# davidmilligan/MLVFS

Measured on AMD Instinct MI355X. Metric: Mpix/s, 3584x1320 14-bit unpack+badpix+cs5x5+stripes (fused, stream resident in HBM), higher is better.
Workload: dtype u16/int32

## Files before the change

### include/mlvfs_amd.h

```cpp
#ifndef MLVFS_AMD_H
#define MLVFS_AMD_H

#include <stddef.h>
#include <stdint.h>
#include <sys/types.h>

#include "mlvfs_abi.h"

#ifdef __cplusplus
extern "C" {
#endif


size_t dng_get_image_data(struct frame_headers *frame_headers, uint16_t *packed_bits,
                          uint8_t *output_buffer, off_t offset, size_t max_size);
size_t dng_get_header_data(struct frame_headers *frame_headers, uint8_t *output_buffer, off_t offset, size_t max_size,
                           double fps_override, char *mlv_basename);
size_t mlvfs_amd_dng_header_lossless(struct frame_headers *frame_headers, uint8_t *output_buffer, off_t offset, size_t max_size,
                                     double fps_override, const char *mlv_basename, uint32_t stream_bytes);
size_t dng_get_header_size(void);
size_t dng_get_image_size(struct frame_headers *frame_headers);
size_t dng_get_size(struct frame_headers *frame_headers);

void chroma_smooth(struct frame_headers *frame_headers, uint16_t *image_data, int method);
// ... 150 lines not shown
int mlvfs_amd_hdr_preview_dev(const mlvfs_amd_geom_t *geom, void *d_frame, size_t max_size, void *stream);

int mlvfs_amd_deflicker_dev(const mlvfs_amd_geom_t *geom, const void *d_frame, size_t size_bytes, int target,
                            int32_t exposure_bias[2], void *stream);

int mlvfs_amd_cr2hdr20_dev(const mlvfs_amd_geom_t *geom, void *d_frame, int interp_method, int fullres, int use_alias_map,
                           int chroma_smooth, void *stream);
int mlvfs_amd_cr2hdr20_batch_dev(const mlvfs_amd_geom_t *geom, void *d_frames, size_t stride, int nframes, int interp_method,
                                 int fullres, int use_alias_map, int chroma_smooth, int *results, void *stream);
void mlvfs_amd_dualiso_reset(void);
void mlvfs_amd_dualiso_trim(void);
void mlvfs_amd_dualiso_last_scalars(double out[8]);

int mlvfs_amd_amaze_demosaic_dev(const float *d_raw, int width, int height, float *d_red, float *d_green, float *d_blue, void *stream);
void mlvfs_amd_amaze_rows_extent(int width, int height, int *nfx, int *nfy);
int mlvfs_amd_amaze_rows_extra_mode(int mode, int width, int height, int *count);
int mlvfs_amd_amaze_debug(const float *d_raw, int width, int height, float *d_red, float *d_green, float *d_blue, int mode,
                          float *d_planes, size_t planes_floats, int *nfx, int *nfy);

int mlvfs_amd_timer_begin(int max_launches);
int mlvfs_amd_timer_end(float *ms, int cap);

int mlvfs_amd_frame_begin(void);
int mlvfs_amd_frame_end(void);
int mlvfs_amd_frame_sync(void *image_data);
void mlvfs_amd_dropin_stats(long long out[2]);
void mlvfs_amd_dropin_transfers(long long out[4]);
void mlvfs_amd_dropin_profile(double out[8]);
void mlvfs_amd_test_fail_next(int what);
int mlvfs_amd_test_rand_layout(void);
int mlvfs_amd_test_device_order(const char *const *bus_ids, int n, int workers, int *device_of);

int mlvfs_amd_test_stream_plan(int width, int height, int seg_rows, int *cols, int *segs, int *fold, int *tasks_per_frame);
int mlvfs_amd_test_frame_plan(const int *in, long long *out);
int mlvfs_amd_test_last_frame_plan(long long out[15]);
int mlvfs_amd_test_stream_listed(void *stream, long long *tiles);
int mlvfs_amd_test_dualiso_parts(int width, int height, int nframes, int *parts, int max_parts, int *tail);

int mlvfs_amd_fix_pattern_noise_dev(const mlvfs_amd_geom_t *geom, void *d_frames, size_t stride, int nframes, void *stream);
size_t mlvfs_amd_test_pn_scratch_cap(size_t bytes);
int mlvfs_amd_deflicker_batch_dev(const mlvfs_amd_geom_t *geom, const void *d_frames, size_t stride, int nframes, size_t size_bytes,
                                  int target, int32_t *exposure_bias, void *stream);
int mlvfs_amd_hdr_preview_batch_dev(const mlvfs_amd_geom_t *geom, void *d_frames, size_t stride, int nframes, size_t max_size,
                                    int *results, void *stream);

typedef struct {
    int32_t chroma_smooth;
    int32_t fix_bad_pixels;
    int32_t fix_stripes;
    int32_t dual_iso;
    int32_t hdr_interpolation_method;
    int32_t hdr_no_fullres;
    int32_t hdr_no_alias_map;
    int32_t deflicker;
    int32_t fix_pattern_noise;
    int32_t rand_mode;
    double fps;
} mlvfs_amd_mount_opts_t;
void *mlvfs_amd_mount_open(const void *reader, const mlvfs_amd_mount_opts_t *opts, const char *mlv_basename);
int mlvfs_amd_mount_dng(void *mount, int first, int count, void *h_out, size_t out_stride, int batch_frames, int io_threads, int *results);
int mlvfs_amd_mount_dng_lossless(void *mount, int first, int count, void *h_out, size_t out_stride, size_t *sizes, int *flags,
                                 int batch_frames, int io_threads, int *results);
void mlvfs_amd_mount_close(void *mount);

typedef struct mlvfs_amd_dark mlvfs_amd_dark_t;
typedef struct mlvfs_amd_look mlvfs_amd_look_t;
typedef struct mlvfs_amd_look16 mlvfs_amd_look16_t;
mlvfs_amd_dark_t *mlvfs_amd_dark_create(const mlvfs_amd_geom_t *geom, const uint16_t *h_plane);
mlvfs_amd_dark_t *mlvfs_amd_dark_from_clip(const void *reader, int first, int count, int batch_frames, int io_threads);
// ... 177 lines not shown
```

### mlvfs_amd/csrc/clip.h

```cpp
#pragma once

#include "common.h"

#include <algorithm>
#include <functional>
#include <memory>
#include <mutex>
#include <vector>

namespace mlv {

constexpr int FRAME_TCW = 64, FRAME_TCH = 15, FRAME_TCH5 = 15, FRAME_HC = 2;
constexpr int FRAME_GEOS = 2;
inline int frame_tile_rows(int geo) { return geo == 1 ? FRAME_TCH5 : FRAME_TCH; }
inline int frame_geo_of(int method) { return method == 5 ? 1 : 0; }
inline int frame_tiles_x(int w) { return (w + 2 * FRAME_TCW - 1) / (2 * FRAME_TCW); }
inline int frame_tiles_y(int h, int geo) { return (h + 2 * frame_tile_rows(geo) - 1) / (2 * frame_tile_rows(geo)); }

struct CellRec {
    int cell;
    int e[4];
};

struct PatchView {
// ... 54 lines not shown
    Geom g{};
    int row0 = 0, row1 = 0, gpr = 0, n_groups = 0, nblk = 0;
    size_t o_counts = 0, o_bsum = 0, o_boff = 0, o_total = 0, o_hist = 0, o_num = 0, o_nre = 0, o_re = 0, o_copies = 0, bytes = 0;
    uint8_t *base = nullptr;
    int init(Clip *owner, const Geom &g, int row0, int row1);
    int count(const void *d_frame, long long *accepted, hipStream_t stream);
    int hist_dev(const void *d_frame, const void *d_rand, long long n_rand, int *d_hist, int *d_num, hipStream_t stream);
    int recheck_into(int32_t *hist_host_or_null, int *d_hist, hipStream_t stream);
    int hist_to_host(const void *d_frame, const void *d_rand, long long n_rand, int32_t *hist, int32_t num[8],
                     hipStream_t stream);
};

struct ThreadCtx;
bool focus_map_applies(struct frame_headers *fh, ThreadCtx *c, int dual_iso);
int focus_pixels_device(struct frame_headers *fh, ThreadCtx *c, void *d_frame, int dual_iso, bool *changed, int *n_patched = nullptr);
int bad_pixels_device(struct frame_headers *fh, ThreadCtx *c, void *d_frame, int aggressive, int dual_iso, bool *changed, int *n_patched = nullptr);

void glibc_rand_stream(uint16_t *out, size_t n, uint64_t skip, unsigned seed);
int stripes_solve(const int32_t *hist, const int32_t num[8], int frame_size, int32_t coeffs[8]);

struct KernelTimer {
    std::vector<hipEvent_t> ev;
    int used = 0;
    bool on = false;
};
KernelTimer &kernel_timer();

int launch_unpack(const void *d_packed, size_t packed_stride, void *d_out, size_t out_stride, uint32_t first_px,
                  uint32_t npix, int bpp, int nframes, hipStream_t stream);
int launch_frame(const Device *dev, const Geom &g, bool packed, const void *src, size_t src_stride, void *dst,
                 size_t dst_stride, int nframes, int method, const PatchView *pv, bool stripes,
                 const int32_t *coef, hipStream_t stream, bool spread = false);
int stream_listed_tiles(hipStream_t stream, long long *tiles);
int dark_share(int packed_bpp, const void *d_frame, int w, int h, int black, hipStream_t stream, int *share_1024);
bool frame_kernel_takes(const Geom &g, const void *src, size_t src_stride, const void *dst, size_t dst_stride, int nframes);
int launch_pixfix(int packed, const void *frames, size_t stride, int w, int black, const void *entries,
                  const int *level_off, int n_levels, int n_level0, int n_entries, void *patches, void *scatter,
                  size_t scatter_stride, int nframes, const DeviceLuts &luts, hipStream_t stream);
int launch_pixfix_for_frame_kernel(int packed, const void *frames, size_t stride, int w, int h, int black, const void *entries,
                                   const int *level_off, int n_levels, int n_level0, int n_entries, void *patches,
                                   const CellRec *recs, int n_rec, void *cells, int nframes, const DeviceLuts &luts, hipStream_t stream);
int launch_pixfix_cells(int packed, const void *frames, size_t stride, int w, int h, const CellRec *recs, int n_rec,
                        const void *patches, int n_entries, void *cells, int nframes, hipStream_t stream);
int launch_deflicker_hist(const void *d_frame, uint32_t samples, uint32_t white, unsigned *d_hist, hipStream_t s);
int launch_deflicker_batch(const void *d_frames, size_t fstride, int nframes, uint32_t samples, uint32_t white, uint32_t middle, unsigned *d_hist,
                           uint16_t *d_med, hipStream_t s);
struct HdrPreviewParams {
    double a, b;
    int dark_row_start, shadow, active, pad;
};
int launch_hdr_row_hist_batch(const void *d_frames, size_t fstride, int nframes, int w, int h, int white, unsigned *d_hist, hipStream_t stream);
int launch_hdr_preview_batch(const void *d_frames, void *d_out, size_t fstride, int nframes, int w, int h, int black, int white,
                             const HdrPreviewParams *d_params, size_t shift_count, hipStream_t stream);
size_t pattern_noise_batch_frame_bytes(int w, int h);
size_t pattern_noise_scratch_cap();
int launch_pattern_noise_batch(void *d_frames, size_t fstride, int nframes, int w, int h, int white, void *d_scratch, size_t scratch_bytes,
                               hipStream_t stream);
int hdr_preview_batch_device(ThreadCtx *c, const Geom &g, void *d_frames, void *d_out, size_t fstride, int nframes, size_t max_size,
                             unsigned *d_hist, HdrPreviewParams *d_params, struct frame_headers *fhs, int *results, hipStream_t stream);
int deflicker_batch_device(const void *d_frames, size_t fstride, int nframes, int bpp, size_t size_bytes, void *d_scratch, size_t scratch_bytes,
                           uint16_t *med, hipStream_t stream);
size_t deflicker_batch_scratch_bytes(int bpp, int nframes);
void deflicker_bias(int target, int black_level, uint16_t median, int32_t exposure_bias[2]);
enum { PAYLOAD_PLAIN = 0, PAYLOAD_LZMA = 1, PAYLOAD_LJ92 = 2 };
inline int payload_kind(uint16_t video_class) { return (video_class & 0x80) ? PAYLOAD_LZMA : (video_class & 0x100) ? PAYLOAD_LJ92 : PAYLOAD_PLAIN; }
struct Calib {
// ... 72 lines not shown
```

### mlvfs_amd/csrc/frame_plan.cpp

```cpp
#include "frame_plan.h"

#include "clip.h"

namespace mlv {

namespace {
constexpr int WGS_PER_CU = 4;
constexpr int RUN_MAX = 22;
constexpr int P5_SEG = 60;
constexpr int S_SEG = 60;

int cus(const FramePassInputs &in) { return in.num_cu > 0 ? in.num_cu : 256; }

int env_switch(const char *name) { const char *e = getenv(name); return e ? atoi(e) : 1; }

bool streamable(const FramePassInputs &in)
{
    return in.packed && in.bpp == 14 && (in.vec == 1 || in.vec == 2) && in.black >= 0 && in.black <= 16384 && in.stripes != StripeForm::generic &&
           in.w >= 16 && in.w % 8 == 0 && in.h >= 2 && in.h % 2 == 0;
}

bool s_takes(const FramePassInputs &in, const FrameSwitches &sw)
{
    if ((in.method != 2 && in.method != 3) || sw.s == 0 || in.pixel_map || !streamable(in)) return false;
    const StreamGeom g = stream_geom(in.w, in.h, S_SEG);
    const long long waves = (long long)cus(in) * WGS_PER_CU * 4;
    return sw.s == 2 || (long long)in.nframes * g.cols * g.segs * 2 >= waves * 7;
}

int p5_seg_rows(const FramePassInputs &in, const FrameSwitches &sw, int grid)
{
    if (in.method != 5 || sw.p5 == 0 || !streamable(in)) return 0;
    const long long cols = stream_geom(in.w, in.h, P5_SEG).cols, rows = in.h / 2;
    const long long waves = (long long)(grid / 4 > 0 ? grid / 4 : 256) * 16;
    for (int seg : { P5_SEG, P5_SEG / 2 })
// ... 38 lines not shown
}

int plan_frame_pass(const FramePassInputs &in, const FrameSwitches &sw, const StreamVerdict &v, FramePlan *out)
{
    if (const int rc = check_frame_pass(in)) return rc;
    FramePlan p;
    const int tiles_x = frame_tiles_x(in.w);
    p.tiles = (long long)tiles_x * frame_tiles_y(in.h, frame_geo_of(in.method)) * in.nframes;

    p.grid = (cus(in) * WGS_PER_CU + 7) / 8 * 8;
    if (p.grid > p.tiles) p.grid = (int)((p.tiles + 7) / 8 * 8);
    const int per_cu = std::min(std::max(p.grid / 4, 1), FRAME_MAX_GROUPS);
    p.groups = per_cu >= 64 ? per_cu / 8 / 8 * 8 : per_cu;
    const int band = (int)(p.tiles / p.groups);
    p.run = std::min(std::max(band / 16, 1), RUN_MAX);
    p.singles = p.run > 1 ? 8 * std::max(p.grid / p.groups, 1) : 0;

    p.watch = frame_pass_watch(in, sw);
    const bool held = p.watch.adaptive && v.held;
    if (p.watch.word == 1 && !held) {
        p.first = FirstKernel::s;
        p.seg_rows = S_SEG;
    } else if (p.watch.word == 0 && !held) {
        p.list_after = true;
        p.seg_rows = v.some_listed && sw.p5 != 2 ? 0 : p5_seg_rows(in, sw, p.grid);
        p.first = p.seg_rows ? FirstKernel::p5 : FirstKernel::p;
        p.first_grid = p.grid;
    }
    if (p.seg_rows) {
        const StreamGeom g = stream_geom(in.w, in.h, p.seg_rows);
        p.cols = g.cols; p.segs = g.segs; p.fold = g.fold;
        p.tasks = (long long)in.nframes * g.tasks_per_frame;
    }
    if (p.first == FirstKernel::s) {
        p.first_grid = cus(in) * WGS_PER_CU;
        if ((long long)p.first_grid * 4 > p.tasks) p.first_grid = (int)((p.tasks + 3) / 4);
        p.steps = (long long)in.nframes * ((p.cols - 1) * p.fold + 1) * (in.h / 2) / p.fold;
    }
    if (p.list_after) {
        long long most = p.tiles;
        if (p.first == FirstKernel::p5) {
            const int full_cols = p.fold > 1 ? p.cols - 1 : p.cols, folded = p.fold > 1 ? (p.segs + p.fold - 1) / p.fold : 0;
            const long long per_frame = (long long)full_cols * p.segs * std::min(tiles_x, tile_cols_spanned(4 * 64)) +
                                        (long long)folded * p.fold * std::min(tiles_x, tile_cols_spanned(4 * 64 / p.fold));
            most = std::max(most, in.nframes * per_frame);
        }
        p.wl_entries = std::max(most, 4096ll);
    }
    *out = p;
    return MLVFS_AMD_OK;
}

namespace {
struct LastPlan { FramePlan plan; bool set = false; };
LastPlan &last_plan() { static thread_local LastPlan t; return t; }

void plan_fields(const FramePlan &p, long long *out)
{
    const long long o[15] = { (long long)p.first, p.list_after, p.grid, p.groups, p.run, p.singles, p.first_grid,
                              p.seg_rows, p.cols, p.segs, p.fold, p.tasks, p.steps, p.wl_entries, p.watch.word };
    for (int i = 0; i < 15; i++) out[i] = o[i];
}
}

void record_frame_plan(const FramePlan &p) { LastPlan &l = last_plan(); l.plan = p; l.set = true; }

}

extern "C" int mlvfs_amd_test_stream_plan(int width, int height, int seg_rows, int *cols, int *segs, int *fold, int *tasks_per_frame)
{
    if (width < 16 || width % 8 || height < 2 || height % 2 || seg_rows < 1 || !cols || !segs || !fold || !tasks_per_frame) return MLVFS_AMD_ERR_ARG;
    const mlv::StreamGeom g = mlv::stream_geom(width, height, seg_rows);
    *cols = g.cols; *segs = g.segs; *fold = g.fold; *tasks_per_frame = g.tasks_per_frame;
    return MLVFS_AMD_OK;
}

extern "C" int mlvfs_amd_test_frame_plan(const int *in, long long *out)
{
    if (!in || !out) return MLVFS_AMD_ERR_ARG;
    const mlv::FramePassInputs fi{ in[0], in[1], in[2], in[3], in[4], in[5] != 0, in[6], in[7] != 0,
                                   in[8] == 2 ? mlv::StripeForm::generic : in[8] == 1 ? mlv::StripeForm::packed : mlv::StripeForm::none,
                                   in[9], in[10] };
    const mlv::StreamVerdict v{ in[11] != 0, in[12] != 0 };
    mlv::FramePlan p;
    if (const int rc = mlv::plan_frame_pass(fi, mlv::frame_switches(), v, &p)) return rc;
    mlv::plan_fields(p, out);
    return MLVFS_AMD_OK;
}

extern "C" int mlvfs_amd_test_stream_listed(void *stream, long long *tiles)
{
    return tiles ? mlv::stream_listed_tiles((hipStream_t)stream, tiles) : MLVFS_AMD_ERR_ARG;
}

extern "C" int mlvfs_amd_test_last_frame_plan(long long *out)
{
    const mlv::LastPlan &l = mlv::last_plan();
    if (!out || !l.set) return MLVFS_AMD_ERR_ARG;
    mlv::plan_fields(l.plan, out);
    return MLVFS_AMD_OK;
}
```

### mlvfs_amd/csrc/frame_plan.h

```cpp
#pragma once

namespace mlv {

constexpr int FRAME_STREAM_COLW = 62;
constexpr int FRAME_MAX_GROUPS = 1024;

enum class FirstKernel { none, p, p5, s };
enum class StripeForm { none, packed, generic };

struct FramePassInputs {
    int w, h, bpp, black;
    int method;
    bool packed;
    int vec;
    bool pixel_map;
    StripeForm stripes;
    int nframes, num_cu;
};

struct FrameSwitches { int p = 1, p5 = 1, s = 1; };
FrameSwitches frame_switches();

struct FrameWatch {
    int word = -1;
    bool adaptive = false;
    bool status = false;
};
FrameWatch frame_pass_watch(const FramePassInputs &in, const FrameSwitches &sw);

struct StreamVerdict {
    bool held = false;
    bool some_listed = false;
};

struct StreamGeom { int cols, segs, fold, tasks_per_frame; };
StreamGeom stream_geom(int w, int h, int seg_rows);

struct FramePlan {
    FirstKernel first = FirstKernel::none;
    bool list_after = false;
    FrameWatch watch;
    long long tiles = 0;
    int grid = 0, groups = 0, run = 0, singles = 0;
    int first_grid = 0;
    int seg_rows = 0, cols = 0, segs = 0, fold = 0;
    long long tasks = 0;
    long long steps = 0;
    long long wl_entries = 0;
};

int check_frame_pass(const FramePassInputs &in);
int plan_frame_pass(const FramePassInputs &in, const FrameSwitches &sw, const StreamVerdict &v, FramePlan *out);

void record_frame_plan(const FramePlan &p);

}
```

### mlvfs_amd/csrc/k_frame.hip

```cpp
#include "frame_plan.h"
#include "k_frame_dev.h"

namespace mlv {

template <int METHOD, bool PACKED, int VEC, bool SPREAD>
__global__ __launch_bounds__(256, 4) void k_frame(const FrameArgs a)
{
    constexpr bool CHAIN = METHOD == 5;
    using Smem = SmemT<SPREAD, CHAIN>;
    __shared__ Smem sm;

    const int list_mode = a.list_mode;
    const int wl_n = list_mode ? cold_args()->wl_ctl[0] : 0;
    auto list_done = [&]() {
        KArgs ka = cold_args();
        int *ctl = ka->wl_ctl, *stat = ka->wl_stat;
        if (atomicAdd(&ctl[2], 1) == min((int)gridDim.x, wl_n) - 1) {
            ctl[0] = 0; ctl[1] = 0; ctl[2] = 0;
            if (stat) { __atomic_store_n(stat, ctl[3], __ATOMIC_RELAXED); __threadfence_system(); }
        }
    };
    if (list_mode && (int)blockIdx.x >= wl_n) {
        if (wl_n == 0 && blockIdx.x == 0 && threadIdx.x == 0) {
            KArgs ka = cold_args();
// ... 375 lines not shown
    if (wt.adaptive && st.h_stat) {
        Backoff &b = st.back[wt.word];
        long long reported = 0, of = 0;
        if (b.look(__atomic_load_n(&st.h_stat[wt.word], __ATOMIC_RELAXED), &reported, &of)) {
            b.judge(reported * 100 > of * (wt.word == 0 ? KF_P_BUSY_PERCENT : KF_S_BUSY_PERCENT));
            if (wt.word == 0) st.some_listed = reported * 100 > of * KF_P5_CALM_PERCENT;
        }
        v.held = b.wide_left > 0;
    }
    v.some_listed = st.some_listed;
    if (const int rc = plan_frame_pass(in, sw, v, pl)) return rc;
    if (wt.adaptive && v.held) st.back[wt.word].wide_left--;
    if (pl->list_after && pl->wl_entries > st.wl_cap) {
        if (st.wl) (void)hipFree(st.wl);
        st.wl = nullptr; st.wl_cap = 0;
        if (hipMalloc(&st.wl, (size_t)pl->wl_entries * sizeof(int2)) != hipSuccess) { set_error("work list: allocation of %lld entries failed", pl->wl_entries); return MLVFS_AMD_ERR_HIP; }
        st.wl_cap = pl->wl_entries;
    }
    if (pl->first == FirstKernel::s) st.back[1].pending += pl->steps;
    if (pl->list_after) st.back[0].pending += pl->tiles;
    *out = st;
    return MLVFS_AMD_OK;
}
int stream_listed_tiles(hipStream_t stream, long long *tiles)
{
    int dev = 0;
    if (hipGetDevice(&dev) != hipSuccess) return MLVFS_AMD_ERR_HIP;
    std::lock_guard<std::mutex> lk(g_ticket_mu);
    const auto it = g_tickets.find({ dev, stream });
    if (it == g_tickets.end() || !it->second.h_stat) return MLVFS_AMD_ERR_ARG;
    *tiles = (long long)(unsigned)__atomic_load_n(&it->second.h_stat[0], __ATOMIC_RELAXED);
    return MLVFS_AMD_OK;
}
void release_stream_state(int device, hipStream_t stream)
{
    std::lock_guard<std::mutex> lk(g_ticket_mu);
    auto it = g_tickets.find({ device, stream });
    if (it == g_tickets.end()) return;
    if (it->second.tickets) (void)hipFree(it->second.tickets);
    if (it->second.wl) (void)hipFree(it->second.wl);
    if (it->second.h_stat) (void)hipHostFree(it->second.h_stat);
    g_tickets.erase(it);
}
__global__ __launch_bounds__(256) void k_build_e2d(const uint16_t *__restrict__ u16, int black, uint2 *__restrict__ e2d, int *__restrict__ bad)
{
    const int b = blockIdx.x * blockDim.x + threadIdx.x;
    if (b >= E2D_RECORDS_EXT) return;
    auto entry = [&](int i) { return (uint16_t)((((int)u16[i & 32767]) >> (13 - (i >> 15))) + black); };
    if (b >= E2D_RECORDS) { e2d[b] = make_uint2(entry(E2R_ENTRIES - 1), 0u); return; }
    unsigned bits = 0;
    uint16_t prev = entry(32 * b);
    const uint16_t base = prev;
    for (int j = 0; j < 31; j++) {
        const uint16_t next = entry(32 * b + j + 1);
        const unsigned d = (uint16_t)(next - prev);
        if (d > 1) atomicAdd(bad, 1);
        bits |= (d & 1u) << j;
        prev = next;
    }
    e2d[b] = make_uint2(base, bits);
}
namespace {
constexpr size_t E2R_CACHE = 8;
struct E2rEntry { uint2 *table; unsigned long long used; };
std::mutex g_tables_mu;
std::map<std::pair<int, int>, E2rEntry> g_e2r;
// ... 179 lines not shown
```

### mlvfs_amd/csrc/k_frame_p.hip

```cpp
#include "frame_plan.h"
#include "k_stream_dev.h"

namespace mlv {

constexpr int P_WAIT_MIN = 1, P_WAIT_MAX = 15;
template <bool SPREAD_>
struct __align__(16) SmemP {
    static constexpr bool SPREAD = SPREAD_;
    uint16_t raw[2 * RH][2 * TCW];
    uint32_t pk[PH][PW];
    int ge[RH][TCW];
    uint16_t t16[MLV_T16_N + (SPREAD_ ? 64 : 0)];
    uint32_t has_patch[PMAP_WORDS];
    uint32_t xchg[3][XCHG_WORDS];
    int unc[2];
    int low[2];
    int dim[2];
    int next_tile, next_end;
    int walk[5];
    int2 carry_at[256];
    uint4 carry_spare;
};

struct PGroup {
// ... 522 lines not shown
            fb_wait = min(2 * fb_wait + 1, P_WAIT_MAX);
            cont = false;
        } else {
            fb_wait = P_WAIT_MIN;
            cont = cont_next;
        }
        low_prev = low_cur;
        t = t_next;
        t_end = t_end_next;
        cur = nxt;
        par ^= 1;
    }
    if (tid == 0) {
        KArgs ka = cold_args();
        const int groups = ka->groups;
        int *tickets = ka->tickets;
        if (atomicAdd(&tickets[2 * groups], 1) == (int)gridDim.x - 1)
            for (int i = 0; i <= 2 * groups; i++) tickets[i] = 0;
    }
}

template <bool SPREAD, int VEC>
__global__ __launch_bounds__(1024, 1) void k_frame_p5(const FrameArgs a, int cols, int segs, int seg_rows, int fold, int S_OUT)
{
    static_assert(!SPREAD, "one table layout");
    asm volatile("" : "+s"(cols));
    constexpr int BPP = 14;
    constexpr int WAVES = 16;
    constexpr int SLOTS = 3;
    constexpr int PARK_LANES = 62;
    struct __align__(16) Smem {
        int ev[MLV_EV32_N];
        uint4 park[WAVES][SLOTS][2][PARK_LANES];
    };
    static_assert(sizeof(Smem) <= 160 * 1024, "the CU's LDS");
    __shared__ Smem sm;
    {
        const uint4 *s4 = (const uint4 *)cold_args()->ev32;
        uint4 *d4 = (uint4 *)sm.ev;
        for (int i = (int)threadIdx.x; i < MLV_EV32_N * 4 / 16; i += 64 * WAVES) d4[i] = s4[i];
    }
    __syncthreads();
    const int lane = (int)threadIdx.x & 63;
    const int w = a.w, h = a.h, black = a.black;
    const uint32_t koff = 4u - 4u * (uint32_t)black;
    const int rows = h >> 1;
    const StreamGrid sg = stream_grid(cols, segs, fold);
    const int ntasks = cold_args()->nframes * sg.per_frame;
    const uint32_t pitch = (uint32_t)(w >> 3) * 14u;
    int *tickets = cold_args()->tickets;
    uint4 (*const mypark)[2][PARK_LANES] = sm.park[threadIdx.x >> 6];
    const int plane = min(max(lane - 1, 0), PARK_LANES - 1);
    const bool parks = lane >= 1 && lane <= PARK_LANES;
    for (;;) {
        const int task = stream_draw(tickets, lane);
        if (task >= ntasks) break;
        const StreamTask t = stream_task<VEC>(task, sg, segs, seg_rows, fold, S_OUT, lane, w, rows);
        const int f = t.f, c = t.c, j0 = t.j0, j1 = t.j1, nparts = t.nparts, P = t.P, roff = t.roff;
        KArgs kt = cold_args();
        const uint8_t *const frame = kt->src + (size_t)f * kt->src_stride;
        const mlv_i32x4 rs_in = frame_rsrc(frame, kt->src_bytes);
        mlv_i32x4 rs_out = { 0, 0, 0, 0 };
        int tx0 = 0;
        bool xm = false;
        uint32_t dA0[4], dA1[4], dB0[4], dB1[4];
        auto issue = [&](int r, uint32_t (&d0)[4], uint32_t (&d1)[4]) { stream_issue(rs_in, r, roff, rows, pitch, t.gbyte, d0, d1); };
        issue(j0 - 2, dA0, dA1);
        issue(j0 - 1, dB0, dB1);
        int ref_r, ref_b;
        {
            const int x0 = min(max(8 * (c * S_OUT + S_OUT / 2), 0), (w - 16) & ~1), y0 = min(j0 + j1, (h - 4) & ~1) & ~1;
            const uint32_t px = fetch_clamped<BPP>(frame, w, h, x0 + (lane & 15), y0 + (lane >> 4));
            const int ev = sm.ev[1 + min(max((int)px - black, 1), 16383)];
            constexpr int CX[5] = { 0, 3, 6, 1, 5 }, CY[5] = { 0, 0, 0, 1, 1 };
            int sdr[5], sdb[5];
#pragma unroll
            for (int k = 0; k < 5; k++) {
                const int l0 = 2 * CX[k] + 32 * CY[k];
                const int rr = __builtin_amdgcn_readlane(ev, l0), g1 = __builtin_amdgcn_readlane(ev, l0 + 1);
                const int g2 = __builtin_amdgcn_readlane(ev, l0 + 16), bb = __builtin_amdgcn_readlane(ev, l0 + 17);
                const int gg = (g1 + g2) >> 1;
                sdr[k] = rr - gg; sdb[k] = bb - gg;
            }
            auto med5 = [](const int (&v)[5]) { return med3i(v[4], max(min(v[0], v[1]), min(v[2], v[3])), min(max(v[0], v[1]), max(v[2], v[3]))); };
            ref_r = med5(sdr);
            ref_b = med5(sdb);
        }
        int n_pm = 0, pm_cell = -1;
// ... 233 lines not shown
```

### mlvfs_amd/csrc/k_stream_dev.h

```cpp
#pragma once
#include "k_frame_dev.h"

namespace mlv {

struct StreamGrid { int ncols_full, nfolded, per_frame; };
__device__ __forceinline__ StreamGrid stream_grid(int cols, int segs, int fold)
{
    StreamGrid sg;
    sg.ncols_full = fold > 1 ? cols - 1 : cols;
    sg.nfolded = fold > 1 ? (segs + fold - 1) / fold : 0;
    sg.per_frame = sg.ncols_full * segs + sg.nfolded;
    return sg;
}

__device__ __forceinline__ int stream_draw(int *tickets, int lane)
{
    int task = 0;
    if (lane == 0) task = atomicAdd(&tickets[0], 1);
    return __builtin_amdgcn_readfirstlane(task);
}

struct StreamTask {
    int f, c;
    int j0, j1;
    int nparts, P;
    int pl, part, roff;
    int g;
    bool writes;
    uint32_t gbyte;
    uint32_t sel, sel1;
};
template <int VEC>
__device__ __forceinline__ StreamTask stream_task(int task, const StreamGrid &sg, int segs, int seg_rows, int fold, int S_OUT, int lane, int w, int rows)
{
    StreamTask t;
    const int gmax = (w >> 3) - 1;
    t.f = task / sg.per_frame;
    const int rem = task - t.f * sg.per_frame;
    const bool folded = rem >= sg.ncols_full * segs;
    t.c = folded ? sg.ncols_full : rem / segs;
    const int seg = folded ? (rem - sg.ncols_full * segs) * fold : rem - t.c * segs;
    t.j0 = seg * seg_rows; t.j1 = min(t.j0 + seg_rows, rows);
    t.nparts = folded ? fold : 1; t.P = folded ? 64 / fold : 64;
    t.pl = lane & (t.P - 1); t.part = folded ? lane / t.P : 0;
    t.roff = t.part * seg_rows;
    const int g_true = t.c * S_OUT + t.pl - 1;
    t.g = min(max(g_true, 0), gmax);
    t.writes = t.pl >= 1 && t.pl <= min(S_OUT, t.P - 2) && g_true <= gmax && t.j0 + t.roff < rows;
    t.gbyte = (uint32_t)t.g * 14u;
    t.sel = (t.g & 1) ? SEL_MIS : SEL_SWAP;
    t.sel1 = VEC == 2 ? t.sel ^ (SEL_SWAP ^ SEL_MIS) : t.sel;
    return t;
// ... 63 lines not shown
```

### mlvfs_amd/lib.py

```python
from __future__ import annotations

import ctypes as C
import os
import subprocess

import numpy as np

from . import abi

HERE = os.path.dirname(os.path.abspath(__file__))
SO_PATH = os.path.join(HERE, "libmlvfs_amd.so")

OK = 0
ERR_HIP, ERR_ARG, ERR_LUT, ERR_NOMEM, ERR_IO = -1, -2, -3, -4, -5
MLV_PLAIN, MLV_LJ92 = 0, 1


class Geom(C.Structure):
    _fields_ = [("width", C.c_int32), ("height", C.c_int32), ("bpp", C.c_int32), ("black", C.c_int32),
                ("white", C.c_int32), ("pan_x", C.c_int32), ("pan_y", C.c_int32)]


class MountOpts(C.Structure):
    _fields_ = [("chroma_smooth", C.c_int32), ("fix_bad_pixels", C.c_int32), ("fix_stripes", C.c_int32), ("dual_iso", C.c_int32),
                ("hdr_interpolation_method", C.c_int32), ("hdr_no_fullres", C.c_int32), ("hdr_no_alias_map", C.c_int32),
                ("deflicker", C.c_int32), ("fix_pattern_noise", C.c_int32), ("rand_mode", C.c_int32), ("fps", C.c_double)]


DROPIN_SYMBOLS = [
    "dng_get_image_data", "dng_get_header_data", "dng_get_header_size", "dng_get_image_size", "dng_get_size",
    "chroma_smooth", "fix_bad_pixels", "fix_focus_pixels", "free_focus_pixel_maps",
    "stripes_get_correction", "stripes_new_correction", "stripes_free_corrections",
    "stripes_compute_correction", "stripes_apply_correction",
    "hdr_convert_data", "cr2hdr20_convert_data", "fix_pattern_noise",
    "hist_create", "hist_add", "hist_median", "hist_destroy", "lj92_open", "lj92_decode", "lj92_close", "lj92_encode", "gif_get_data", "gif_get_size",
]
DEVICE_SYMBOLS = [
    "mlvfs_amd_device_count", "mlvfs_amd_device_pci_bus_id", "mlvfs_amd_thread_device", "mlvfs_amd_init", "mlvfs_amd_last_error", "mlvfs_amd_version",
    "mlvfs_amd_clip_create", "mlvfs_amd_clip_destroy", "mlvfs_amd_clip_set_stripes", "mlvfs_amd_clip_get_stripes",
    "mlvfs_amd_clip_set_pixel_map", "mlvfs_amd_clip_get_pixel_map", "mlvfs_amd_clip_set_t16_layout", "mlvfs_amd_clip_get_t16_layout",
    "mlvfs_amd_unpack_dev", "mlvfs_amd_chroma_smooth_dev", "mlvfs_amd_detect_bad_pixels_dev",
    "mlvfs_amd_fix_pixels_dev", "mlvfs_amd_stripes_count_dev", "mlvfs_amd_stripes_hist_dev",
    "mlvfs_amd_stripes_solve", "mlvfs_amd_stripes_compute_dev", "mlvfs_amd_stripes_apply_dev",
    "mlvfs_amd_rand_stream", "mlvfs_amd_rand_stream_dev", "mlvfs_amd_process_frames_dev", "mlvfs_amd_process_frames_host",
    "mlvfs_amd_host_alloc", "mlvfs_amd_host_free", "mlvfs_amd_host_owns", "mlvfs_amd_host_size", "mlvfs_amd_host_knows", "mlvfs_amd_host_trim", "mlvfs_amd_hdr_preview_dev",
    "mlvfs_amd_cr2hdr20_dev", "mlvfs_amd_cr2hdr20_batch_dev", "mlvfs_amd_dualiso_reset", "mlvfs_amd_dualiso_trim", "mlvfs_amd_dualiso_last_scalars", "mlvfs_amd_amaze_demosaic_dev", "mlvfs_amd_amaze_debug", "mlvfs_amd_amaze_rows_extent", "mlvfs_amd_amaze_rows_extra_mode",
    "mlvfs_amd_timer_begin", "mlvfs_amd_timer_end", "mlvfs_amd_selftest_host", "mlvfs_amd_selftest_tables", "mlvfs_amd_test_median_net", "mlvfs_amd_frame_begin", "mlvfs_amd_frame_end", "mlvfs_amd_frame_sync", "mlvfs_amd_dropin_stats", "mlvfs_amd_test_fail_next", "mlvfs_amd_dropin_transfers", "mlvfs_amd_dropin_profile",
    "mlvfs_amd_mlv_open", "mlvfs_amd_mlv_close", "mlvfs_amd_mlv_frame_count", "mlvfs_amd_mlv_chunk_count",
    "mlvfs_amd_mlv_xref", "mlvfs_amd_mlv_frame_headers", "mlvfs_amd_mlv_read_frames", "mlvfs_amd_mlv_process", "mlvfs_amd_mlv_process_dualiso",
    "mlvfs_amd_lj92_info", "mlvfs_amd_lj92_decode_dev", "mlvfs_amd_lj92_decode_untiled", "mlvfs_amd_lj92_encode_table", "mlvfs_amd_test_rand_layout", "mlvfs_amd_test_device_order", "mlvfs_amd_test_stream_plan", "mlvfs_amd_test_lj92_row_plan", "mlvfs_amd_test_lj92_encode_plan", "mlvfs_amd_test_frame_plan", "mlvfs_amd_test_last_frame_plan", "mlvfs_amd_test_stream_listed", "mlvfs_amd_test_dualiso_parts", "mlvfs_amd_lzma_uncompress",
    "mlvfs_amd_gif_size", "mlvfs_amd_gif_render", "mlvfs_amd_mlv_gif_data", "mlvfs_amd_process_unpacked_dev", "mlvfs_amd_deflicker_dev",
    "mlvfs_amd_fix_pattern_noise_dev", "mlvfs_amd_test_pn_scratch_cap", "mlvfs_amd_deflicker_batch_dev", "mlvfs_amd_hdr_preview_batch_dev",
    "mlvfs_amd_mount_open", "mlvfs_amd_mount_dng", "mlvfs_amd_mount_close",
    "mlvfs_amd_lj92_encode_batch_dev", "mlvfs_amd_dng_header_lossless", "mlvfs_amd_mount_dng_lossless",
    "mlvfs_amd_lj92_tile_dev", "mlvfs_amd_pack_dev", "mlvfs_amd_mlv_transcode",
    "mlvfs_amd_dark_create", "mlvfs_amd_dark_from_clip", "mlvfs_amd_dark_info", "mlvfs_amd_dark_plane", "mlvfs_amd_dark_destroy",
    "mlvfs_amd_dark_subtract_dev", "mlvfs_amd_mount_set_dark", "mlvfs_amd_mlv_transcode_dark",
    "mlvfs_amd_rawi_set_bits", "mlvfs_amd_repack_dev", "mlvfs_amd_mlv_transcode_bits",
    "mlvfs_amd_flat_create", "mlvfs_amd_flat_from_clip", "mlvfs_amd_flat_info", "mlvfs_amd_flat_gain", "mlvfs_amd_flat_destroy",
    "mlvfs_amd_flat_apply_dev", "mlvfs_amd_mount_set_flat", "mlvfs_amd_mlv_transcode_cal",
    "mlvfs_amd_proxy_geom", "mlvfs_amd_bin2_dev", "mlvfs_amd_dng_header_proxy", "mlvfs_amd_mount_set_proxy", "mlvfs_amd_mount_dng_size",
    "mlvfs_amd_rgb_geom", "mlvfs_amd_rgb_header_size", "mlvfs_amd_rgb_lut", "mlvfs_amd_rgb_params", "mlvfs_amd_rgb_header",
    "mlvfs_amd_render2_dev", "mlvfs_amd_mount_rgb", "mlvfs_amd_mount_rgb_size",
    "mlvfs_amd_jpeg_header_size", "mlvfs_amd_jpeg_header", "mlvfs_amd_jpeg_qtables", "mlvfs_amd_jpeg_scratch_bytes",
    "mlvfs_amd_jpeg_encode_dev", "mlvfs_amd_mount_jpeg",
    "mlvfs_amd_rgb_full_geom", "mlvfs_amd_render1_dev", "mlvfs_amd_mount_rgb_full", "mlvfs_amd_mount_jpeg_full", "mlvfs_amd_mount_rgb_full_size",
    "mlvfs_amd_rgb_fit", "mlvfs_amd_render_scaled_dev", "mlvfs_amd_mount_rgb_scaled", "mlvfs_amd_mount_jpeg_scaled",
    "mlvfs_amd_mount_rgb_scaled_size", "mlvfs_amd_test_scale_div", "mlvfs_amd_test_scale_plan",
    "mlvfs_amd_look_image_size", "mlvfs_amd_look_pack", "mlvfs_amd_look_create", "mlvfs_amd_look_destroy", "mlvfs_amd_look_apply_dev",
    "mlvfs_amd_render2_look_dev", "mlvfs_amd_render1_look_dev", "mlvfs_amd_render_scaled_look_dev", "mlvfs_amd_mount_set_look",
    "mlvfs_amd_look16_image_size", "mlvfs_amd_look16_pack", "mlvfs_amd_look16_create", "mlvfs_amd_look16_destroy", "mlvfs_amd_look16_apply_dev",
    "mlvfs_amd_rgb16_header", "mlvfs_amd_render2_deep_dev", "mlvfs_amd_render1_deep_dev", "mlvfs_amd_render_scaled_deep_dev",
    "mlvfs_amd_mount_rgb16", "mlvfs_amd_mount_rgb16_full", "mlvfs_amd_mount_rgb16_scaled",
    "mlvfs_amd_mount_rgb16_size", "mlvfs_amd_mount_rgb16_full_size", "mlvfs_amd_mount_rgb16_scaled_size",
    "mlvfs_amd_rgb_fit_full", "mlvfs_amd_render_resampled_dev", "mlvfs_amd_render_resampled_look_dev", "mlvfs_amd_render_resampled_deep_dev",
    "mlvfs_amd_mount_rgb_resampled", "mlvfs_amd_mount_jpeg_resampled", "mlvfs_amd_mount_rgb16_resampled",
    "mlvfs_amd_mount_rgb_resampled_size", "mlvfs_amd_mount_rgb16_resampled_size", "mlvfs_amd_test_resample_plan",
    "mlvfs_amd_rgb_amaze_geom", "mlvfs_amd_amaze_balance_dev", "mlvfs_amd_amaze_tone_dev", "mlvfs_amd_render1_amaze_dev",
    "mlvfs_amd_render1_amaze_look_dev", "mlvfs_amd_render1_amaze_deep_dev", "mlvfs_amd_mount_set_demosaic", "mlvfs_amd_test_amaze_render_plan",
    "mlvfs_amd_rgb_amaze_resample_geom", "mlvfs_amd_amaze_resample_dev", "mlvfs_amd_render_resampled_amaze_dev",
    "mlvfs_amd_render_resampled_amaze_look_dev", "mlvfs_amd_render_resampled_amaze_deep_dev", "mlvfs_amd_mount_set_resample_demosaic",
    "mlvfs_amd_test_amz_resample_plan",
    "mlvfs_amd_jpeg_header_sampled", "mlvfs_amd_jpeg_scratch_bytes_sampled", "mlvfs_amd_jpeg_mcus", "mlvfs_amd_jpeg_encode_sampled_dev",
# ... 87 lines not shown
    sig("mlvfs_amd_stripes_apply_dev", i, [vp, vp, sz, i, vp])
    sig("mlvfs_amd_rand_stream", None, [vp, sz, C.c_uint64, C.c_uint])
    sig("mlvfs_amd_rand_stream_dev", i, [vp, sz, C.c_uint64, C.c_uint, vp])
    sig("mlvfs_amd_process_frames_dev", i, [vp, vp, sz, vp, sz, i, i, i, i, vp])
    sig("mlvfs_amd_process_frames_host", i, [vp, vp, sz, vp, sz, i, i, i, i, i])
    sig("mlvfs_amd_host_alloc", vp, [sz])
    sig("mlvfs_amd_host_free", None, [vp])
    sig("mlvfs_amd_host_owns", i, [vp, sz])
    sig("mlvfs_amd_host_size", sz, [vp])
    sig("mlvfs_amd_host_knows", i, [vp])
    sig("mlvfs_amd_host_trim", sz, [])
    sig("mlvfs_amd_hdr_preview_dev", i, [gp, vp, sz, vp])
    sig("mlvfs_amd_cr2hdr20_dev", i, [gp, vp, i, i, i, i, vp])
    sig("mlvfs_amd_cr2hdr20_batch_dev", i, [gp, vp, sz, i, i, i, i, i, vp, vp])
    sig("mlvfs_amd_dualiso_reset", None, [])
    sig("mlvfs_amd_dualiso_trim", None, [])
    sig("mlvfs_amd_dualiso_last_scalars", None, [vp])
    sig("mlvfs_amd_amaze_demosaic_dev", i, [vp, i, i, vp, vp, vp, vp])
    sig("mlvfs_amd_amaze_rows_extent", None, [i, i, C.POINTER(C.c_int), C.POINTER(C.c_int)])
    sig("mlvfs_amd_amaze_rows_extra_mode", i, [i, i, i, C.POINTER(C.c_int)])
    sig("mlvfs_amd_amaze_debug", i, [vp, i, i, vp, vp, vp, i, vp, sz, C.POINTER(C.c_int), C.POINTER(C.c_int)])
    sig("mlvfs_amd_timer_begin", i, [i])
    sig("mlvfs_amd_timer_end", i, [vp, i])
    sig("mlvfs_amd_selftest_host", i, [])
    sig("mlvfs_amd_selftest_tables", i, [vp, vp])
    sig("mlvfs_amd_test_median_net", i, [i, i, vp, vp])
    sig("mlvfs_amd_frame_begin", i, [])
    sig("mlvfs_amd_frame_end", i, [])
    sig("mlvfs_amd_frame_sync", i, [vp])
    sig("mlvfs_amd_dropin_stats", None, [vp])
    sig("mlvfs_amd_test_fail_next", None, [C.c_int])
    sig("mlvfs_amd_test_device_order", i, [vp, i, i, vp])
    sig("mlvfs_amd_test_stream_plan", i, [i, i, i, vp, vp, vp, vp])
    sig("mlvfs_amd_test_lj92_row_plan", i, [i, i, vp])
    sig("mlvfs_amd_test_lj92_encode_plan", i, [C.c_longlong, vp])
    sig("mlvfs_amd_test_frame_plan", i, [vp, vp])
    sig("mlvfs_amd_test_last_frame_plan", i, [vp])
    sig("mlvfs_amd_test_stream_listed", i, [vp, vp])
    sig("mlvfs_amd_test_dualiso_parts", i, [i, i, i, vp, i, vp])
    sig("mlvfs_amd_dropin_transfers", None, [vp])
    sig("mlvfs_amd_dropin_profile", None, [vp])
    sig("mlvfs_amd_process_unpacked_dev", i, [vp, vp, sz, vp, sz, i, i, i, i, vp])
    sig("mlvfs_amd_deflicker_dev", i, [gp, vp, sz, i, vp, vp])
    sig("mlvfs_amd_lzma_uncompress", i, [vp, sz, vp, sz, C.POINTER(sz)])
    sig("mlvfs_amd_gif_size", sz, [fhp])
    sig("mlvfs_amd_gif_render", i, [gp, vp, sz, i, i, vp])
    sig("mlvfs_amd_mlv_gif_data", sz, [vp, vp, C.c_long, sz])
    sig("mlvfs_amd_lj92_info", i, [vp, sz, vp])
    sig("mlvfs_amd_lj92_decode_dev", i, [vp, vp, i, i, i, vp, sz, vp])
    sig("mlvfs_amd_mlv_open", vp, [C.c_char_p, i])
    sig("mlvfs_amd_mlv_close", None, [vp])
    sig("mlvfs_amd_mlv_frame_count", i, [vp])
    sig("mlvfs_amd_mlv_chunk_count", i, [vp])
    sig("mlvfs_amd_mlv_xref", sz, [vp, vp, sz])
    sig("mlvfs_amd_mlv_frame_headers", i, [vp, i, fhp])
    sig("mlvfs_amd_mlv_read_frames", i, [vp, i, i, vp, sz, i])
    sig("mlvfs_amd_mlv_process", i, [vp, vp, i, i, vp, sz, i, i, i, i, i])
    sig("mlvfs_amd_mlv_process_dualiso", i, [vp, i, i, vp, sz, i, i, i, i, i, i, vp])
    sig("mlvfs_amd_fix_pattern_noise_dev", i, [gp, vp, sz, i, vp])
    sig("mlvfs_amd_test_pn_scratch_cap", sz, [sz])
    sig("mlvfs_amd_deflicker_batch_dev", i, [gp, vp, sz, i, sz, i, vp, vp])
    sig("mlvfs_amd_hdr_preview_batch_dev", i, [gp, vp, sz, i, sz, vp, vp])
    sig("mlvfs_amd_mount_open", vp, [vp, C.POINTER(MountOpts), C.c_char_p])
    sig("mlvfs_amd_mount_dng", i, [vp, i, i, vp, sz, i, i, vp])
    sig("mlvfs_amd_mount_close", None, [vp])
    sig("mlvfs_amd_lj92_encode_batch_dev", i, [vp, sz, i, i, i, i, vp, sz, vp, vp, vp, vp])
    sig("mlvfs_amd_dng_header_lossless", sz, [fhp, vp, C.c_long, sz, C.c_double, C.c_char_p, C.c_uint32])
    sig("mlvfs_amd_mount_dng_lossless", i, [vp, i, i, vp, sz, vp, vp, i, i, vp])
    sig("mlvfs_amd_lj92_tile_dev", i, [vp, sz, vp, sz, i, i, i, vp])
    sig("mlvfs_amd_pack_dev", i, [gp, vp, sz, vp, sz, i, vp])
    sig("mlvfs_amd_mlv_transcode", i, [vp, C.c_char_p, i, i, i, C.POINTER(C.c_longlong)])
# ... 120 lines not shown
```

Measured before the change: 971,700.

## Hand out stream tasks in static per-workgroup blocks, then dynamic tickets

```diff
diff --git a/include/mlvfs_amd.h b/include/mlvfs_amd.h
--- a/include/mlvfs_amd.h
+++ b/include/mlvfs_amd.h
@@ -206,9 +206,12 @@
 int mlvfs_amd_test_device_order(const char *const *bus_ids, int n, int workers, int *device_of);
 
 int mlvfs_amd_test_stream_plan(int width, int height, int seg_rows, int *cols, int *segs, int *fold, int *tasks_per_frame);
+int mlvfs_amd_test_stream_order(int width, int height, int seg_rows, int frames, int workgroups, long long *info, int *order_to_task,
+                                int *static_tasks, long long room);
 int mlvfs_amd_test_frame_plan(const int *in, long long *out);
 int mlvfs_amd_test_last_frame_plan(long long out[15]);
 int mlvfs_amd_test_stream_listed(void *stream, long long *tiles);
+int mlvfs_amd_test_stream_worklist(void *stream, long long tiles, int *entries, long long room, long long *n);
 int mlvfs_amd_test_dualiso_parts(int width, int height, int nframes, int *parts, int max_parts, int *tail);
 
 int mlvfs_amd_fix_pattern_noise_dev(const mlvfs_amd_geom_t *geom, void *d_frames, size_t stride, int nframes, void *stream);
diff --git a/mlvfs_amd/csrc/clip.h b/mlvfs_amd/csrc/clip.h
--- a/mlvfs_amd/csrc/clip.h
+++ b/mlvfs_amd/csrc/clip.h
@@ -110,6 +110,7 @@
                  size_t dst_stride, int nframes, int method, const PatchView *pv, bool stripes,
                  const int32_t *coef, hipStream_t stream, bool spread = false);
 int stream_listed_tiles(hipStream_t stream, long long *tiles);
+int stream_worklist(hipStream_t stream, long long tiles, int *entries, long long room, long long *n);
 int dark_share(int packed_bpp, const void *d_frame, int w, int h, int black, hipStream_t stream, int *share_1024);
 bool frame_kernel_takes(const Geom &g, const void *src, size_t src_stride, const void *dst, size_t dst_stride, int nframes);
 int launch_pixfix(int packed, const void *frames, size_t stride, int w, int black, const void *entries,
diff --git a/mlvfs_amd/csrc/frame_plan.cpp b/mlvfs_amd/csrc/frame_plan.cpp
--- a/mlvfs_amd/csrc/frame_plan.cpp
+++ b/mlvfs_amd/csrc/frame_plan.cpp
@@ -1,6 +1,7 @@
 #include "frame_plan.h"
 
 #include "clip.h"
+#include "k_stream_order.h"
 
 namespace mlv {
 
@@ -105,6 +106,7 @@
         p.cols = g.cols; p.segs = g.segs; p.fold = g.fold;
         p.tasks = (long long)in.nframes * g.tasks_per_frame;
     }
+    if (p.first == FirstKernel::p5) p.static_rounds = stream_static_rounds(p.tasks, (p.first_grid + 3) / 4);
     if (p.first == FirstKernel::s) {
         p.first_grid = cus(in) * WGS_PER_CU;
         if ((long long)p.first_grid * 4 > p.tasks) p.first_grid = (int)((p.tasks + 3) / 4);
@@ -148,6 +150,28 @@
     return MLVFS_AMD_OK;
 }
 
+extern "C" int mlvfs_amd_test_stream_order(int width, int height, int seg_rows, int frames, int workgroups, long long *info, int *order_to_task,
+                                           int *static_tasks, long long room)
+{
+    if (width < 16 || width % 8 || height < 2 || height % 2 || seg_rows < 1 || frames < 1 || workgroups < 1 || !info) return MLVFS_AMD_ERR_ARG;
+    const mlv::StreamGeom g = mlv::stream_geom(width, height, seg_rows);
+    const long long tasks = (long long)frames * g.tasks_per_frame;
+    if (tasks >= (1ll << 31)) return MLVFS_AMD_ERR_ARG;
+    const int ncols_full = g.fold > 1 ? g.cols - 1 : g.cols, rounds = mlv::stream_static_rounds(tasks, workgroups);
+    info[0] = tasks; info[1] = rounds; info[2] = mlv::stream_dynamic_start(rounds, workgroups);
+    if (order_to_task)
+        for (long long n = 0; n < tasks; n++) order_to_task[n] = mlv::stream_order_task((int)n, ncols_full, g.segs, g.fold, g.tasks_per_frame);
+    if (static_tasks) {
+        const int per_wg = rounds * mlv::STREAM_BLOCK;
+        if ((long long)workgroups * per_wg > room) return MLVFS_AMD_ERR_ARG;
+        for (int wg = 0; wg < workgroups; wg++)
+            for (int k = 0; k < per_wg; k++)
+                static_tasks[(long long)wg * per_wg + k] =
+                    mlv::stream_order_task(mlv::stream_static_number(k, wg, workgroups), ncols_full, g.segs, g.fold, g.tasks_per_frame);
+    }
+    return MLVFS_AMD_OK;
+}
+
 extern "C" int mlvfs_amd_test_frame_plan(const int *in, long long *out)
 {
     if (!in || !out) return MLVFS_AMD_ERR_ARG;
@@ -166,6 +190,11 @@
     return tiles ? mlv::stream_listed_tiles((hipStream_t)stream, tiles) : MLVFS_AMD_ERR_ARG;
 }
 
+extern "C" int mlvfs_amd_test_stream_worklist(void *stream, long long tiles, int *entries, long long room, long long *n)
+{
+    return entries && n && tiles >= 0 && room >= 0 ? mlv::stream_worklist((hipStream_t)stream, tiles, entries, room, n) : MLVFS_AMD_ERR_ARG;
+}
+
 extern "C" int mlvfs_amd_test_last_frame_plan(long long *out)
 {
     const mlv::LastPlan &l = mlv::last_plan();
diff --git a/mlvfs_amd/csrc/frame_plan.h b/mlvfs_amd/csrc/frame_plan.h
--- a/mlvfs_amd/csrc/frame_plan.h
+++ b/mlvfs_amd/csrc/frame_plan.h
@@ -45,6 +45,7 @@
     int first_grid = 0;
     int seg_rows = 0, cols = 0, segs = 0, fold = 0;
     long long tasks = 0;
+    int static_rounds = 0;
     long long steps = 0;
     long long wl_entries = 0;
 };
diff --git a/mlvfs_amd/csrc/k_frame.hip b/mlvfs_amd/csrc/k_frame.hip
--- a/mlvfs_amd/csrc/k_frame.hip
+++ b/mlvfs_amd/csrc/k_frame.hip
@@ -431,6 +431,28 @@
     *tiles = (long long)(unsigned)__atomic_load_n(&it->second.h_stat[0], __ATOMIC_RELAXED);
     return MLVFS_AMD_OK;
 }
+int stream_worklist(hipStream_t stream, long long tiles, int *entries, long long room, long long *n)
+{
+    int dev = 0;
+    if (hipGetDevice(&dev) != hipSuccess) return MLVFS_AMD_ERR_HIP;
+    std::vector<int2> host;
+    {
+        std::lock_guard<std::mutex> lk(g_ticket_mu);
+        const auto it = g_tickets.find({ dev, stream });
+        if (it == g_tickets.end()) return MLVFS_AMD_ERR_ARG;
+        host.resize((size_t)it->second.wl_cap);
+        if (!host.empty() && hipMemcpy(host.data(), it->second.wl, host.size() * sizeof(int2), hipMemcpyDeviceToHost) != hipSuccess) return MLVFS_AMD_ERR_HIP;
+    }
+    long long sum = 0, k = 0;
+    while (sum < tiles && k < (long long)host.size() && k < room) {
+        if (host[(size_t)k].y <= 0) return MLVFS_AMD_ERR_ARG;
+        entries[2 * k] = host[(size_t)k].x; entries[2 * k + 1] = host[(size_t)k].y;
+        sum += host[(size_t)k].y; k++;
+    }
+    if (sum != tiles) return MLVFS_AMD_ERR_ARG;
+    *n = k;
+    return MLVFS_AMD_OK;
+}
 void release_stream_state(int device, hipStream_t stream)
 {
     std::lock_guard<std::mutex> lk(g_ticket_mu);
diff --git a/mlvfs_amd/csrc/k_frame_p.hip b/mlvfs_amd/csrc/k_frame_p.hip
--- a/mlvfs_amd/csrc/k_frame_p.hip
+++ b/mlvfs_amd/csrc/k_frame_p.hip
@@ -578,6 +578,7 @@
     struct __align__(16) Smem {
         int ev[MLV_EV32_N];
         uint4 park[WAVES][SLOTS][2][PARK_LANES];
+        int draw;
     };
     static_assert(sizeof(Smem) <= 160 * 1024, "the CU's LDS");
     __shared__ Smem sm;
@@ -585,6 +586,7 @@
         const uint4 *s4 = (const uint4 *)cold_args()->ev32;
         uint4 *d4 = (uint4 *)sm.ev;
         for (int i = (int)threadIdx.x; i < MLV_EV32_N * 4 / 16; i += 64 * WAVES) d4[i] = s4[i];
+        if (threadIdx.x == 0) sm.draw = 0;
     }
     __syncthreads();
     const int lane = (int)threadIdx.x & 63;
@@ -595,11 +597,12 @@
     const int ntasks = cold_args()->nframes * sg.per_frame;
     const uint32_t pitch = (uint32_t)(w >> 3) * 14u;
     int *tickets = cold_args()->tickets;
+    const int static_rounds = stream_static_rounds(ntasks, (int)gridDim.x);
     uint4 (*const mypark)[2][PARK_LANES] = sm.park[threadIdx.x >> 6];
     const int plane = min(max(lane - 1, 0), PARK_LANES - 1);
     const bool parks = lane >= 1 && lane <= PARK_LANES;
     for (;;) {
-        const int task = stream_draw(tickets, lane);
+        const int task = stream_draw_blocks(&sm.draw, tickets, lane, ntasks, static_rounds, sg, segs, fold);
         if (task >= ntasks) break;
         const StreamTask t = stream_task<VEC>(task, sg, segs, seg_rows, fold, S_OUT, lane, w, rows);
         const int f = t.f, c = t.c, j0 = t.j0, j1 = t.j1, nparts = t.nparts, P = t.P, roff = t.roff;
diff --git a/mlvfs_amd/csrc/k_stream_dev.h b/mlvfs_amd/csrc/k_stream_dev.h
--- a/mlvfs_amd/csrc/k_stream_dev.h
+++ b/mlvfs_amd/csrc/k_stream_dev.h
@@ -1,5 +1,6 @@
 #pragma once
 #include "k_frame_dev.h"
+#include "k_stream_order.h"
 
 namespace mlv {
 
@@ -18,6 +19,19 @@
     int task = 0;
     if (lane == 0) task = atomicAdd(&tickets[0], 1);
     return __builtin_amdgcn_readfirstlane(task);
+}
+
+__device__ __forceinline__ int stream_draw_blocks(int *lds_draw, int *tickets, int lane, int ntasks, int static_rounds, const StreamGrid &sg, int segs, int fold)
+{
+    int n = 0;
+    if (lane == 0) {
+        const int wgs = (int)gridDim.x;
+        const int k = atomicAdd(lds_draw, 1);
+        n = (k >> 4) < static_rounds ? stream_static_number(k, (int)blockIdx.x, wgs)
+                                     : (int)stream_dynamic_start(static_rounds, wgs) + atomicAdd(&tickets[0], 1);
+    }
+    n = __builtin_amdgcn_readfirstlane(n);
+    return n < ntasks ? stream_order_task(n, sg.ncols_full, segs, fold, sg.per_frame) : n;
 }
 
 struct StreamTask {
diff --git a/mlvfs_amd/csrc/k_stream_order.h b/mlvfs_amd/csrc/k_stream_order.h
--- /dev/null
+++ b/mlvfs_amd/csrc/k_stream_order.h
@@ -0,0 +1,44 @@
+#pragma once
+
+#if defined(__HIPCC__) || defined(__CUDACC__)
+#define MLV_ORDER_FN __host__ __device__ inline
+#else
+#define MLV_ORDER_FN inline
+#endif
+
+namespace mlv {
+
+constexpr int STREAM_BLOCK = 16;
+
+MLV_ORDER_FN int stream_order_task(int n, int ncols_full, int segs, int fold, int per_frame)
+{
+    const int f = n / per_frame, r = n - f * per_frame;
+    int rem;
+    if (fold > 1) {
+        const int per_group = fold * ncols_full + 1, grp = r / per_group, q = r - grp * per_group;
+        if (q == ncols_full) rem = ncols_full * segs + grp;
+        else {
+            const int q1 = q < ncols_full ? q : q - 1, s = q1 / ncols_full;
+            rem = (q1 - s * ncols_full) * segs + grp * fold + s;
+        }
+    } else {
+        const int s = r / ncols_full;
+        rem = (r - s * ncols_full) * segs + s;
+    }
+    return f * per_frame + rem;
+}
+
+MLV_ORDER_FN int stream_static_rounds(long long tasks, int workgroups)
+{
+    const long long rounds = tasks / ((long long)workgroups * STREAM_BLOCK);
+    return rounds > 1 ? (int)(rounds - 1) : 0;
+}
+
+MLV_ORDER_FN int stream_static_number(int k, int workgroup, int workgroups)
+{
+    return ((k >> 4) * workgroups + workgroup) * STREAM_BLOCK + (k & (STREAM_BLOCK - 1));
+}
+
+MLV_ORDER_FN long long stream_dynamic_start(int static_rounds, int workgroups) { return (long long)static_rounds * workgroups * STREAM_BLOCK; }
+
+}
diff --git a/mlvfs_amd/lib.py b/mlvfs_amd/lib.py
--- a/mlvfs_amd/lib.py
+++ b/mlvfs_amd/lib.py
@@ -48,7 +48,7 @@
     "mlvfs_amd_timer_begin", "mlvfs_amd_timer_end", "mlvfs_amd_selftest_host", "mlvfs_amd_selftest_tables", "mlvfs_amd_test_median_net", "mlvfs_amd_frame_begin", "mlvfs_amd_frame_end", "mlvfs_amd_frame_sync", "mlvfs_amd_dropin_stats", "mlvfs_amd_test_fail_next", "mlvfs_amd_dropin_transfers", "mlvfs_amd_dropin_profile",
     "mlvfs_amd_mlv_open", "mlvfs_amd_mlv_close", "mlvfs_amd_mlv_frame_count", "mlvfs_amd_mlv_chunk_count",
     "mlvfs_amd_mlv_xref", "mlvfs_amd_mlv_frame_headers", "mlvfs_amd_mlv_read_frames", "mlvfs_amd_mlv_process", "mlvfs_amd_mlv_process_dualiso",
-    "mlvfs_amd_lj92_info", "mlvfs_amd_lj92_decode_dev", "mlvfs_amd_lj92_decode_untiled", "mlvfs_amd_lj92_encode_table", "mlvfs_amd_test_rand_layout", "mlvfs_amd_test_device_order", "mlvfs_amd_test_stream_plan", "mlvfs_amd_test_lj92_row_plan", "mlvfs_amd_test_lj92_encode_plan", "mlvfs_amd_test_frame_plan", "mlvfs_amd_test_last_frame_plan", "mlvfs_amd_test_stream_listed", "mlvfs_amd_test_dualiso_parts", "mlvfs_amd_lzma_uncompress",
+    "mlvfs_amd_lj92_info", "mlvfs_amd_lj92_decode_dev", "mlvfs_amd_lj92_decode_untiled", "mlvfs_amd_lj92_encode_table", "mlvfs_amd_test_rand_layout", "mlvfs_amd_test_device_order", "mlvfs_amd_test_stream_plan", "mlvfs_amd_test_stream_order", "mlvfs_amd_test_lj92_row_plan", "mlvfs_amd_test_lj92_encode_plan", "mlvfs_amd_test_frame_plan", "mlvfs_amd_test_last_frame_plan", "mlvfs_amd_test_stream_listed", "mlvfs_amd_test_stream_worklist", "mlvfs_amd_test_dualiso_parts", "mlvfs_amd_lzma_uncompress",
     "mlvfs_amd_gif_size", "mlvfs_amd_gif_render", "mlvfs_amd_mlv_gif_data", "mlvfs_amd_process_unpacked_dev", "mlvfs_amd_deflicker_dev",
     "mlvfs_amd_fix_pattern_noise_dev", "mlvfs_amd_test_pn_scratch_cap", "mlvfs_amd_deflicker_batch_dev", "mlvfs_amd_hdr_preview_batch_dev",
     "mlvfs_amd_mount_open", "mlvfs_amd_mount_dng", "mlvfs_amd_mount_close",
@@ -202,11 +202,13 @@
     sig("mlvfs_amd_test_fail_next", None, [C.c_int])
     sig("mlvfs_amd_test_device_order", i, [vp, i, i, vp])
     sig("mlvfs_amd_test_stream_plan", i, [i, i, i, vp, vp, vp, vp])
+    sig("mlvfs_amd_test_stream_order", i, [i, i, i, i, i, vp, vp, vp, C.c_longlong])
     sig("mlvfs_amd_test_lj92_row_plan", i, [i, i, vp])
     sig("mlvfs_amd_test_lj92_encode_plan", i, [C.c_longlong, vp])
     sig("mlvfs_amd_test_frame_plan", i, [vp, vp])
     sig("mlvfs_amd_test_last_frame_plan", i, [vp])
     sig("mlvfs_amd_test_stream_listed", i, [vp, vp])
+    sig("mlvfs_amd_test_stream_worklist", i, [vp, C.c_longlong, vp, C.c_longlong, vp])
     sig("mlvfs_amd_test_dualiso_parts", i, [i, i, i, vp, i, vp])
     sig("mlvfs_amd_dropin_transfers", None, [vp])
     sig("mlvfs_amd_dropin_profile", None, [vp])
```

After: 960,500. 1.1% lower.
